# BenChung/SuccessiveConvexification

Measured on AMD Instinct MI355X. Metric: 6-DoF K=50 SCvx iterations/sec (batch), higher is better.
Workload: dtype f64

## Files before the change

successiveconvexification_amd/csrc/scvx_ipm_core.hpp:

```cpp
#pragma once
#include <math.h>
#include <stdint.h>
#include <type_traits>

#if defined(__HIPCC__)
#define SCVX_HD __host__ __device__ __forceinline__
#define SCVX_HD_NI __host__ __device__ __attribute__((noinline))
#else
#define SCVX_HD inline
#define SCVX_HD_NI inline
#endif
#if defined(SCVX_IPM_PROF) && defined(__HIP_DEVICE_COMPILE__)
#define SCVX_TS(v) const unsigned long long v = __builtin_amdgcn_s_memtime()
#define SCVX_TE(v, slot) prof[slot] += (double)(__builtin_amdgcn_s_memtime() - v)
#else
#define SCVX_TS(v)
#define SCVX_TE(v, slot)
#endif
#ifndef SCVX_NODE_QR
#define SCVX_NODE_QR 0
#endif
#ifndef SCVX_STALL_ITERS
#define SCVX_STALL_ITERS 3
#endif
// ... 342 lines not shown
    int status;
    int iters;
    double merit, pobj;
    int warmed;
    int attempts;
};

template <class Ex, class Stor = double, class DStor = Stor, int NU = 3, class FStor = SCVX_FACTOR_T>
struct Solver {
    static_assert(NU == 3 || NU == 5, "control_dim 3 (the reference's live model) or 5 (fin extension)");
    static constexpr int NP = 14 + 2 * NU + 1;
    static constexpr int DSZ = 14 * NP;
    static constexpr int CS = 14 + 2 * NU;
    static constexpr int NXU = 14 + NU;
    static constexpr int HU_SZ = hu_size(NU);
    static constexpr int NODE_SZ = HX_SZ + HU_SZ;
    static constexpr int TW = 14 + 2 * NU;
    static constexpr int TS = NU == 5 ? 26 : 22;
    static constexpr int BPN = 14 * NU;
    static constexpr int NPW = (DSZ + 63) / 64;
    typedef typename gp<Stor>::ptr gptr;
    typedef typename gp<Stor>::cptr cgptr;
    typedef typename gp<DStor>::ptr dptr;
    typedef typename gp<DStor>::cptr dcptr;
    typedef typename gp<double>::cptr cdptr;
    typedef typename gp<FStor>::ptr fptr;
    typedef typename gp<FStor>::cptr cfptr;
    Ex& ex;
    const Consts& C;
    Layout L;
    cdptr xbar, ubar, endpoint;
    dcptr D;
    double rk;
    gptr dk, V, rx, gx, dw, r1, cw, Vbest, tmpv;
    gptr y, ry, dy, r2, cy, tmpy, tmpy2, rp, tq0, tq1;
    gptr S, Z, lam, Wv, Wibz, tmpc, Wirz, sd;
    gptr Wbeta;
    gptr hx, hu;
    fptr Linv, Nf;
    gptr tchain;
    dptr At;
    gptr ys, ytr, ynu;
    gptr ptl, rtr;
    gptr tmpl, tmpl2;
    gptr uhat, lb0;
    gptr wh, Vw, yw, Sw, Zw;
    double h_tr[4], h_nu[4], hrk, hnui;
    double q_tr[2], q_nu[2], q_sg[4], h00s;
    double css, cst, csn, cts, ctt, ctn, cns, cnt_, pny;
    double p_step_frac = SCVX_STEP_FRAC, p_init_shift = SCVX_INIT_SHIFT, p_init_balance = SCVX_INIT_BALANCE;
    bool p_sigma_cube = false;
    double p_mu_floor = 0.25;
    double bigvz[2];
    double bigs[2][6];
    bool bigs_ok;
    double bigvv[2];
    double bigq[2][6];
    double res_nrx2, res_nry2, res_sgy;
    bool tsp;
    double gram[16];
    double gn_pred;
    double bigvx2[2];
#if defined(SCVX_IPM_PROF)
    double prof[32];
#endif
    double cur_gate;

    SCVX_HD Solver(Ex& e, const Consts& c) : ex(e), C(c) {
        L.init(c.K, c.vmax > 0.0, NU);
#if defined(SCVX_IPM_PROF)
        for (int i = 0; i < 32; i++) prof[i] = 0.0;
#endif
    }

    SCVX_HD void carve(gptr w) {
        const int nv = L.nv, ny = L.ny, nc = L.nc, nloc = L.nloc, K = L.K;
        dk = w; w += ny;
        V = w; w += nv; rx = w; w += nv; gx = w; w += nv; dw = w; w += nv; r1 = w; w += nv; cw = w; w += nv;
        Vbest = w; w += nv; tmpv = w; w += nv;
        y = w; w += ny; ry = w; w += ny; dy = w; w += ny; r2 = w; w += ny; cy = w; w += ny; tmpy = w; w += ny; tmpy2 = w; w += ny; rp = w; w += ny; tq0 = w; w += ny; tq1 = w; w += ny;
        S = w; w += nc; Z = w; w += nc; lam = w; w += nc; Wv = w; w += nc;
        Wibz = w; w += nc; tmpc = w; w += nc; Wirz = w; w += nc; sd = w; w += nc;
        Wbeta = w; w += L.ncones;
        hx = w; w += (size_t)(K + 1) * HX_SZ; hu = w; w += (size_t)(K + 1) * HU_SZ;
        Linv = (fptr)w; w += (size_t)K * LINV_SZ; Nf = (fptr)w; w += (size_t)K * 196; At = (dptr)w; w += (size_t)K * 196;
        tchain = w; w += ny;
        ys = w; w += ny; ytr = w; w += ny; ynu = w; w += ny; rtr = w; w += ny; ptl = w; w += nloc;
        tmpl = w; w += nloc; tmpl2 = w; w += nloc;
        uhat = w; w += 3 * (K + 1); lb0 = w; w += (K + 1);
        w += 64;
        wh = w; w += 8; Vw = w; w += nv; yw = w; w += ny; Sw = w; w += nc; Zw = w; w += nc;
    }

    SCVX_HD bool fixed_x(int k, int j) const {
        if (k == 0) return !(j >= 7 && j < 11);
        if (k == L.K) return j != 0;
        return false;
    }
    SCVX_HD bool fixed_u(int k, int c) const { return k == L.K && (c == 1 || c == 2); }

    template <class PH>
    static SCVX_HD double bhu(const double* Dt, int c0, int i, int c, PH h) {
        if (NU == 3 || c < 3) return Dt[14 * c0 + i] * h[c] + Dt[14 * (c0 + 1) + i] * h[3 + c] + Dt[14 * (c0 + 2) + i] * h[6 + c];
        return Dt[14 * (c0 + 3) + i] * h[9 + (c - 3)] + Dt[14 * (c0 + 4) + i] * h[11 + (c - 3)];
    }
    static SCVX_HD double so_elem(const double* T, const double* Bp, int i, int j) {
        double a = -T[TS * i + j];
        SCVX_UNROLL
// ... 294 lines not shown
        each_small<4>(L.o_dp, L.c_dp, L.ndp, f);
        if (with_sg) { each_small<2>(L.o_sg, L.c_sg, 1, f); each_small<1>(L.o_rk, L.c_rk, 1, f); }
    }

    SCVX_HD void identity_scaling() {
        for (int i = ex.lane(); i < L.nc; i += ex.nlanes()) Wv[i] = 0.0;
        ex.sync();
        all_small([&](auto, int off, int c) { Wv[off] = 1.0; Wbeta[c] = 1.0; }, false);
        if (ex.lane() == 0) {
            Wv[L.o_nu] = 1.0; Wv[L.o_tr] = 1.0; Wv[L.o_sg] = 1.0; Wv[L.o_rk] = 1.0;
            Wbeta[L.c_nu] = Wbeta[L.c_tr] = Wbeta[L.c_sg] = Wbeta[L.c_rk] = 1.0;
        }
        bigvv[0] = bigvv[1] = 0.0;
        ex.sync();
    }
    SCVX_HD_NI void W_all(cgptr in, gptr out, bool inverse) {
        SCVX_THIS_LDS();
        SCVX_T0();
        all_small([&](auto Dt_, int off, int c) {
            constexpr int d = decltype(Dt_)::value;
            const double beta = Wbeta[c];
            if (d == 1) out[off] = inverse ? in[off] / beta : in[off] * beta;
            else {
                double xv[d], vv[d], yv[d];
                for (int i = 0; i < d; i++) { xv[i] = in[off + i]; vv[i] = Wv[off + i]; }
                soc_W_small(vv, beta, d, xv, yv, inverse);
                for (int i = 0; i < d; i++) out[off + i] = yv[i];
            }
        }, true);
        big_W(L.o_nu, 14 * L.K + 1, L.c_nu, in, out, inverse);
        big_W(L.o_tr, NXU * (L.K + 1) + 1, L.c_tr, in, out, inverse);
        ex.sync();
        SCVX_T1(8);
    }
    enum { G_GS3 = 0, G_RATE = 1, G_MASS = 2, G_T4 = 3, G_LB = 4, G_SG = 5, G_RK = 6, G_DP = 7, G_FIN = 8 };
    template <int GRP, int D, class F>
    SCVX_HD void each_small_g(int off0, int c0, int n, F&& f) {
        for (int q = ex.lane(); q < n; q += ex.nlanes())
            f(std::integral_constant<int, GRP>(), std::integral_constant<int, D>(), off0 + D * q, c0 + q, q);
    }
    template <class F>
    SCVX_HD void for_small(F&& f) {
        const int K = L.K;
        each_small_g<G_GS3, 3>(L.o_gs, L.c_gs, 2 * K, f);
        each_small_g<G_RATE, 4>(L.o_rate, L.c_rate, K, f);
        each_small_g<G_MASS, 1>(L.o_mass, L.c_mass, K, f);
        each_small_g<G_T4, 4>(L.o_tb, L.c_tb, 2 * (K + 1), f);
        each_small_g<G_LB, 1>(L.o_lb, L.c_lb, K + 1, f);
        if constexpr (NU == 5) each_small_g<G_FIN, 3>(L.o_fin, L.c_fin, L.nfin, f);
        each_small_g<G_DP, 4>(L.o_dp, L.c_dp, L.ndp, f);
        each_small_g<G_SG, 2>(L.o_sg, L.c_sg, 1, f);
        each_small_g<G_RK, 1>(L.o_rk, L.c_rk, 1, f);
    }
    template <int GRP, int D>
    SCVX_HD void small_gather(int q, cgptr v, double af, double (&o)[D]) const {
        const int K = L.K;
        if constexpr (GRP == G_GS3) {
            const bool gs = q < K;
            const int k = gs ? q : q - K;
            cgptr dx = v + 14 * k; cdptr xb = xbar + 14 * k;
            const int i1 = gs ? 2 : 9, i2 = gs ? 3 : 10;
            const double x1 = af * xb[1] + dx[1];
            o[0] = gs ? x1 * C.itan : af * C.sqcm;
            o[1] = af * xb[i1] + dx[i1];
            o[2] = af * xb[i2] + dx[i2];
        } else if constexpr (GRP == G_RATE) {
            cgptr dx = v + 14 * q; cdptr xb = xbar + 14 * q;
            o[0] = af * C.omMax;
            for (int j = 0; j < 3; j++) o[1 + j] = af * xb[11 + j] + dx[11 + j];
        } else if constexpr (GRP == G_MASS) {
            const int k = q + 1;
            o[0] = (af * xbar[14 * k] + v[14 * k]) - af * C.mdry;
        } else if constexpr (GRP == G_T4) {
            const bool tb = q <= K;
            const int k = tb ? q : q - (K + 1);
            cgptr du = v + L.nx + NU * k; cdptr ub = ubar + NU * k;
            double u[3];
            for (int c = 0; c < 3; c++) u[c] = af * ub[c] + du[c];
            o[0] = tb ? af * C.Tmax : u[0] * C.icos;
            o[1] = u[0]; o[2] = u[1]; o[3] = u[2];
        } else if constexpr (GRP == G_LB) {
            cgptr du = v + L.nx + NU * q;
            o[0] = uhat[3 * q] * du[0] + uhat[3 * q + 1] * du[1] + uhat[3 * q + 2] * du[2] - af * lb0[q];
        } else if constexpr (GRP == G_FIN) {
            cgptr du = v + L.nx + NU * q; cdptr ub = ubar + NU * q;
            o[0] = af * C.finmxf;
            o[1] = af * ub[3] + du[3];
            o[2] = af * ub[4] + du[4];
        } else if constexpr (GRP == G_DP) {
            cgptr dx = v + 14 * q; cdptr xb = xbar + 14 * q;
            o[0] = af * C.vmax;
            for (int j = 0; j < 3; j++) o[1 + j] = af * xb[4 + j] + dx[4 + j];
        } else if constexpr (GRP == G_SG) {
            o[0] = v[L.iTS]; o[1] = v[L.iS];
        } else {
            o[0] = af * rk - v[L.iTTR];
        }
    }
    struct BigCone { int off, dim, cidx, head, body; };
    SCVX_HD BigCone big_cone(int q) const {
        return q == 0 ? BigCone{L.o_nu, 14 * L.K + 1, L.c_nu, L.iTNU, L.nx + L.nu_}
                      : BigCone{L.o_tr, NXU * (L.K + 1) + 1, L.c_tr, L.iTTR, 0};
    }
    struct D6 { double a, b, c, d, e, f; };

    SCVX_HD_NI void scale_pass(double& gap_out, double& nrz2_out) {
        SCVX_THIS_LDS();
        SCVX_T0();
        double gap = 0, nrz2 = 0;
        const cgptr S_ = S; const cgptr Z_ = Z; const cgptr V_ = V;
        const gptr Wv_ = Wv; const gptr lam_ = lam; const gptr Wirz_ = Wirz; const gptr tmpc_ = tmpc; const gptr Wbeta_ = Wbeta;
        for_small([&](auto G_, auto Dt_, int off, int c, int q) {
            constexpr int GRP = decltype(G_)::value, D = decltype(Dt_)::value;
            double s[D], z[D], a[D], r[D];
            for (int i = 0; i < D; i++) { s[i] = S_[off + i]; z[i] = Z_[off + i]; }
            small_gather<GRP, D>(q, V_, 1.0, a);
            for (int i = 0; i < D; i++) { r[i] = s[i] - a[i]; gap += s[i] * z[i]; nrz2 += r[i] * r[i]; }
            if constexpr (D == 1) {
                const double beta = sqrt(s[0] / z[0]), l = sqrt(s[0] * z[0]);
                const double wr = r[0] / beta;
                Wbeta_[c] = beta; Wv_[off] = 1.0; lam_[off] = l; Wirz_[off] = wr; tmpc_[off] = (l - wr) / beta;
            } else {
                double beta, v[D], l[D], wr[D], m[D], t[D];
                soc_nt_small(s, z, D, v, beta);
                soc_W_small(v, beta, D, z, l, false);
                soc_W_small(v, beta, D, r, wr, true);
                for (int i = 0; i < D; i++) m[i] = l[i] - wr[i];
                soc_W_small(v, beta, D, m, t, true);
                Wbeta_[c] = beta;
                for (int i = 0; i < D; i++) { Wv_[off + i] = v[i]; lam_[off + i] = l[i]; Wirz_[off + i] = wr[i]; tmpc_[off + i] = t[i]; }
            }
        });
        for (int q = 0; q < 2; q++) {
            const BigCone bc = big_cone(q);
            const cgptr s = S_ + bc.off; const cgptr z = Z_ + bc.off; const cgptr ab = V_ + bc.body - 1;
            double a = 0, b = 0, c = 0;
            const bool carried = SCVX_CARRY_BIGSUMS != 0 && bigs_ok;
            if (carried) { a = bigs[q][0]; b = bigs[q][1]; c = bigs[q][2]; }
            else {
                stream(1, bc.dim, [&](int i) { return D2{s[i], z[i]}; },
                       [&](int, const D2& v) { a += v.a * v.a; b += v.b * v.b; c += v.a * v.b; });
                a = ex.sum(a); b = ex.sum(b); c = ex.sum(c);
            }
            const double s0 = s[0], z0 = z[0], r0 = s0 - V_[bc.head];
            const double sj = sqrt(s0 * s0 - a), zj = sqrt(z0 * z0 - b);
            const double isj = 1.0 / sj, izj = 1.0 / zj;
            const double gam = sqrt(0.5 * (1.0 + (s0 * z0 + c) * isj * izj));
            const double ig = 0.5 / gam;
            const double wb0 = (s0 * isj + z0 * izj) * ig;
            const double den = 1.0 / sqrt(2.0 * (wb0 + 1.0));
            const double v0 = (wb0 + 1.0) * den, beta = sqrt(sj * izj), ibeta = 1.0 / beta;
            const double igd = ig * den;
            double vz = 0, vr = 0, vv = 0, g1 = 0, n1 = 0;
            if (carried) {
                const double sr = bigs[q][3], zr = bigs[q][4];
                vz = (c * isj - b * izj) * igd;
                vr = (sr * isj - zr * izj) * igd;
                vv = ((a * isj) * isj - 2.0 * (c * isj) * izj + (b * izj) * izj) * (igd * igd);
                if (ex.lane() == 0) { gap += c; nrz2 += bigs[q][5]; }
            } else {
            stream(1, bc.dim, [&](int i) { return D3{s[i], z[i], ab[i]}; },
                   [&](int, const D3& w) {
                       const double vi = (w.a * isj - w.b * izj) * igd, ri = w.a - w.c;
                       vz += vi * w.b; vr += vi * ri; vv += vi * vi; g1 += w.a * w.b; n1 += ri * ri;
                   });
            vz = ex.sum(vz); vr = ex.sum(vr); vv = ex.sum(vv);
            }
            bigvv[q] = vv;
            gap += g1; nrz2 += n1;
            if (ex.lane() == 0) { gap += s0 * z0; nrz2 += r0 * r0; }
            const double vxz = v0 * z0 + vz;
            const double l0 = (2.0 * vxz * v0 - z0) * beta;
            const double vxr = v0 * r0 - vr;
            const double wr0 = (2.0 * vxr * v0 - r0) * ibeta;
            const double m0 = l0 - wr0;
            const double vl = beta * (2.0 * vxz * vv + vz);
            const double vw = (-2.0 * vxr * vv + vr) * ibeta;
            const double vxm = v0 * m0 - (vl - vw);
            const double t0 = (2.0 * vxm * v0 - m0) * ibeta;
            const gptr vo = Wv_ + bc.off; const gptr lo = lam_ + bc.off; const gptr wo = Wirz_ + bc.off; const gptr to = tmpc_ + bc.off;
            stream(1, bc.dim, [&](int i) { return D3{s[i], z[i], ab[i]}; },
                   [&](int i, const D3& w) {
                       const double vi = (w.a * isj - w.b * izj) * igd, ri = w.a - w.c;
                       const double li = (2.0 * vxz * vi + w.b) * beta;
                       const double wi = (-2.0 * vxr * vi + ri) * ibeta;
                       vo[i] = vi; lo[i] = li; wo[i] = wi;
                       to[i] = (-2.0 * vxm * vi + (li - wi)) * ibeta;
                   });
            if (ex.lane() == 0) { vo[0] = v0; lo[0] = l0; wo[0] = wr0; to[0] = t0; Wbeta_[bc.cidx] = beta; }
        }
        ex.sync();
        gap_out = ex.sum(gap);
        nrz2_out = ex.sum(nrz2);
        SCVX_T1(11);
    }

    template <bool PRED, bool CHECK = false>
    SCVX_HD_NI double dir_pass() {
        static_assert(!(PRED && CHECK), "the operator-form check belongs to the corrector");
        SCVX_THIS_LDS();
        SCVX_T0();
        double amax = INFINITY;
        const cgptr dw_ = dw; const cgptr Wv_ = Wv; const cgptr lam_ = lam; const cgptr Wirz_ = Wirz; const cgptr Wibz_ = Wibz;
        const cgptr Wbeta_ = Wbeta; const gptr sd_ = sd; const gptr tc_ = tmpc;
        for_small([&](auto G_, auto Dt_, int off, int c, int q) {
            constexpr int GRP = decltype(G_)::value, D = decltype(Dt_)::value;
            double ds[D], l[D], wr[D], a[D], b[D];
            small_gather<GRP, D>(q, dw_, 0.0, ds);
            const double beta = Wbeta_[c];
            for (int i = 0; i < D; i++) { l[i] = lam_[off + i]; wr[i] = Wirz_[off + i]; }
            if constexpr (D == 1) {
                const double wij = ds[0] / beta;
                if (CHECK) tc_[off] = wij / beta;
                a[0] = wij - wr[0];
                b[0] = PRED ? -l[0] - a[0] : -(wij + Wibz_[off]);
                const double sa = a[0] < 0.0 ? -l[0] / a[0] : INFINITY, sb = b[0] < 0.0 ? -l[0] / b[0] : INFINITY;
                if (sa < amax) amax = sa;
                if (sb < amax) amax = sb;
            } else {
                double v[D], wij[D];
                for (int i = 0; i < D; i++) v[i] = Wv_[off + i];
                soc_W_small(v, beta, D, ds, wij, true);
                if (CHECK) {
                    double uu[D];
                    soc_W_small(v, beta, D, wij, uu, true);
                    for (int i = 0; i < D; i++) tc_[off + i] = uu[i];
                }
                for (int i = 0; i < D; i++) { a[i] = wij[i] - wr[i]; b[i] = PRED ? -l[i] - a[i] : -(wij[i] + Wibz_[off + i]); }
                double ll = 0, la = 0, aa = 0, lb = 0, bb = 0;
                for (int i = 1; i < D; i++) { ll += l[i] * l[i]; la += l[i] * a[i]; aa += a[i] * a[i]; lb += l[i] * b[i]; bb += b[i] * b[i]; }
                const double sa = soc_maxstep_parts(l[0], a[0], l[0] * l[0] - ll, l[0] * a[0] - la, a[0] * a[0] - aa);
                const double sb = soc_maxstep_parts(l[0], b[0], l[0] * l[0] - ll, l[0] * b[0] - lb, b[0] * b[0] - bb);
                if (sa < amax) amax = sa;
                if (sb < amax) amax = sb;
            }
            for (int i = 0; i < D; i++) sd_[off + i] = PRED ? a[i] : b[i];
        });
        amax = ex.min(amax);
        for (int q = 0; q < 2; q++) {
            const BigCone bc = big_cone(q);
            const cgptr v = Wv_ + bc.off; const cgptr l = lam_ + bc.off; const cgptr wr = Wirz_ + bc.off; const cgptr wb = Wibz_ + bc.off;
            const cgptr db = dw_ + bc.body - 1;
            const gptr so = sd_ + bc.off;
            double vd = 0;
            stream(1, bc.dim, [&](int i) { return D2{v[i], db[i]}; }, [&](int, const D2& w) { vd += w.a * w.b; });
            vd = ex.sum(vd);
            const double beta = Wbeta_[bc.cidx], ibeta = 1.0 / beta, v0 = v[0], d0 = dw_[bc.head], l0 = l[0];
// ... 51 lines not shown
        const gptr Wibz_ = Wibz; const gptr tmpc_ = tmpc;
        for_small([&](auto, auto Dt_, int off, int c, int) {
            constexpr int D = decltype(Dt_)::value;
            double l[D], a[D], b[D], wr[D];
            for (int i = 0; i < D; i++) { l[i] = lam_[off + i]; a[i] = sd_[off + i]; wr[i] = Wirz_[off + i]; b[i] = -l[i] - a[i]; }
            const double beta = Wbeta_[c];
            if constexpr (D == 1) {
                const double rhs = -l[0] * l[0] + (-a[0] * b[0] + sigmu);
                const double wb = -wr[0] - rhs / l[0];
                Wibz_[off] = wb; tmpc_[off] = wb / beta;
            } else {
                double rhs[D], t[D], wb[D], v[D], o[D];
                double ll = 0, ab = 0;
                for (int i = 0; i < D; i++) { ll += l[i] * l[i]; ab += a[i] * b[i]; }
                for (int i = 1; i < D; i++) rhs[i] = -2.0 * l[0] * l[i] - (a[0] * b[i] + b[0] * a[i]);
                rhs[0] = -ll + (-ab + sigmu);
                double ld = 0, l1 = 0;
                for (int i = 1; i < D; i++) { ld += l[i] * rhs[i]; l1 += l[i] * l[i]; }
                const double x0 = (l[0] * rhs[0] - ld) / (l[0] * l[0] - l1);
                const double il0 = 1.0 / l[0];
                t[0] = x0;
                for (int i = 1; i < D; i++) t[i] = (rhs[i] - x0 * l[i]) * il0;
                for (int i = 0; i < D; i++) { wb[i] = -wr[i] - t[i]; v[i] = Wv_[off + i]; }
                soc_W_small(v, beta, D, wb, o, true);
                for (int i = 0; i < D; i++) { Wibz_[off + i] = wb[i]; tmpc_[off + i] = o[i]; }
            }
        });
        for (int q = 0; q < 2; q++) {
            const BigCone bc = big_cone(q);
            const cgptr v = Wv_ + bc.off; const cgptr l = lam_ + bc.off; const cgptr wr = Wirz_ + bc.off; const cgptr a = sd_ + bc.off;
            const gptr wbo = Wibz_ + bc.off; const gptr to = tmpc_ + bc.off;
            const double l0 = l[0], a0 = a[0], b0 = -l0 - a0, v0 = v[0], wr0 = wr[0];
            const double beta = Wbeta_[bc.cidx], ibeta = 1.0 / beta;
            const double c1 = -2.0 * l0 + a0, c2 = a0 - b0;
            const double ll = bigq[q][0], la = bigq[q][1], aa = bigq[q][2], vl = bigq[q][3], vw = bigq[q][4], va = bigq[q][5];
            const double ab = -la - aa, lr = c1 * ll + c2 * la, vr = c1 * vl + c2 * va;
            const double rhs0 = -(ll + l0 * l0) + (-(ab + a0 * b0) + sigmu);
            const double x0 = (l0 * rhs0 - lr) / (l0 * l0 - ll);
            const double il0 = 1.0 / l0;
            const double wb0 = -wr0 - x0;
            const double vt = (vr - x0 * vl) * il0;
            const double vx = v0 * wb0 - (-vw - vt);
            stream(1, bc.dim, [&](int i) { return D4{l[i], a[i], v[i], wr[i]}; },
                   [&](int i, const D4& w) {
                       const double bi = -w.a - w.b, ri = -2.0 * l0 * w.a - (a0 * bi + b0 * w.b);
                       const double wbi = -w.d - (ri - x0 * w.a) * il0;
                       wbo[i] = wbi;
                       to[i] = (-2.0 * vx * w.c + wbi) * ibeta;
                   });
            if (ex.lane() == 0) { wbo[0] = wb0; to[0] = (2.0 * vx * v0 - wb0) * ibeta; }
        }
        ex.sync();
        SCVX_T1(22);
    }

    SCVX_HD_NI void update_pass(double alpha, gptr Vn) {
        SCVX_THIS_LDS();
        SCVX_T0();
        const gptr S_ = S; const gptr Z_ = Z; const cgptr V_ = V; const cgptr dw_ = dw; const cgptr Wv_ = Wv; const cgptr sd_ = sd;
        const cgptr Wbeta_ = Wbeta;
        for_small([&](auto G_, auto Dt_, int off, int c, int q) {
            constexpr int GRP = decltype(G_)::value, D = decltype(Dt_)::value;
            double s[D], z[D], a[D], jd[D], b[D];
            for (int i = 0; i < D; i++) { s[i] = S_[off + i]; z[i] = Z_[off + i]; b[i] = sd_[off + i]; }
            small_gather<GRP, D>(q, V_, 1.0, a);
            small_gather<GRP, D>(q, dw_, 0.0, jd);
            const double beta = Wbeta_[c];
            if constexpr (D == 1) {
                S_[off] = s[0] + alpha * (jd[0] - (s[0] - a[0]));
                Z_[off] = z[0] + alpha * (b[0] / beta);
            } else {
                double v[D], dz[D];
                for (int i = 0; i < D; i++) v[i] = Wv_[off + i];
                soc_W_small(v, beta, D, b, dz, true);
                for (int i = 0; i < D; i++) { S_[off + i] = s[i] + alpha * (jd[i] - (s[i] - a[i])); Z_[off + i] = z[i] + alpha * dz[i]; }
            }
        });
        for (int q = 0; q < 2; q++) {
            const BigCone bc = big_cone(q);
            const gptr s = S_ + bc.off; const gptr z = Z_ + bc.off; const cgptr v = Wv_ + bc.off; const cgptr b = sd_ + bc.off;
            const cgptr ab = V_ + bc.body - 1; const cgptr db = dw_ + bc.body - 1;
            const double beta = Wbeta_[bc.cidx], ibeta = 1.0 / beta, v0 = v[0], b0 = b[0];
            const double vx = v0 * b0 - bigvz[q];
            const double s0 = s[0], z0 = z[0], a0 = V_[bc.head], d0 = dw_[bc.head];
            ex.sync();
            const gptr vnb = Vn + bc.body - 1;
            double q0 = 0, q1 = 0, q2 = 0, q3 = 0, q4 = 0, q5 = 0;
            stream(1, bc.dim, [&](int i) { return D6{s[i], z[i], v[i], b[i], ab[i], db[i]}; },
                   [&](int i, const D6& w) {
                       const double sn = w.a + alpha * (w.f - (w.a - w.e));
                       const double zn = w.b + alpha * ((-2.0 * vx * w.c + w.d) * ibeta);
                       const double vn = w.e + alpha * w.f;
                       s[i] = sn; z[i] = zn; vnb[i] = vn;
                       const double rn = sn - vn;
                       q0 += sn * sn; q1 += zn * zn; q2 += sn * zn; q3 += sn * rn; q4 += zn * rn; q5 += rn * rn;
                   });
            bigs[q][0] = ex.sum(q0); bigs[q][1] = ex.sum(q1); bigs[q][2] = ex.sum(q2);
            bigs[q][3] = ex.sum(q3); bigs[q][4] = ex.sum(q4); bigs[q][5] = ex.sum(q5);
            if (ex.lane() == 0) {
                s[0] = s0 + alpha * (d0 - (s0 - a0));
                z[0] = z0 + alpha * ((2.0 * vx * v0 - b0) * ibeta);
            }
        }
        ex.sync();
        for (int i = L.nloc + ex.lane(); i < L.nv; i += ex.nlanes()) Vn[i] = V_[i] + alpha * dw_[i];
        bigs_ok = true;
        {
            const gptr y_ = y; const cgptr dy_ = dy;
            stream(0, L.ny, [&](int i) { return D2{y_[i], dy_[i]}; }, [&](int i, const D2& v) { y_[i] = v.a + alpha * v.b; });
        }
        ex.sync();
        SCVX_T1(23);
    }

    SCVX_HD_NI void Hb_inv(cgptr g, gptr out, bool with_nu = true) {
        SCVX_THIS_LDS();
        SCVX_T0();
        const int K = L.K;
        const cgptr hx_ = hx; const cgptr hu_ = hu;
        stream(0, L.nx,
               [&](int t) {
                   const int k = t / 14, j = t - 14 * k;
                   const int hb = j == 0 ? HX_M : j < 4 ? HX_R + 3 * (j - 1) : j < 7 ? HX_V + 3 * (j - 4) : j < 9 ? HX_Q
                                  : j < 11 ? HX_Q34 + 2 * (j - 9) : HX_W + 3 * (j - 11);
                   const int gb = j == 0 ? 0 : j < 4 ? 1 : j < 7 ? 4 : j < 9 ? j : j < 11 ? 9 : 11;
                   const int n = (j == 0 || j == 7 || j == 8) ? 1 : (j == 9 || j == 10) ? 2 : 3;
                   cgptr h = hx_ + (size_t)k * HX_SZ + hb; cgptr x = g + 14 * k + gb;
                   const int i1 = n > 1 ? 1 : 0, i2 = n > 2 ? 2 : 0;
                   return D6{h[0], n > 1 ? h[i1] : 0.0, n > 2 ? h[i2] : 0.0, x[0], x[i1], x[i2]};
               },
               [&](int t, const D6& w) { out[t] = w.a * w.d + w.b * w.e + w.c * w.f; });
        {
            cgptr gu = g + L.nx; gptr ou = out + L.nx;
            stream(0, L.nu_,
                   [&](int t) {
                       const int k = t / NU, c = t - NU * k;
                       if (NU == 3 || c < 3) { cgptr h = hu_ + HU_SZ * k + 3 * c; cgptr x = gu + NU * k; return D6{h[0], h[1], h[2], x[0], x[1], x[2]}; }
                       cgptr h = hu_ + HU_SZ * k + 9 + 2 * (c - 3); cgptr x = gu + NU * k + 3;
                       return D6{h[0], h[1], 0.0, x[0], x[1], 0.0};
                   },
                   [&](int t, const D6& w) { ou[t] = w.a * w.d + w.b * w.e + w.c * w.f; });
        }
        if (with_nu) {
            cgptr gn = g + L.nx + L.nu_; gptr on = out + L.nx + L.nu_;
            const double hn = hnui;
            stream<8>(0, 14 * K, [&](int i) { return gn[i]; }, [&](int i, double v) { on[i] = hn * v; });
        }
        ex.sync();
        SCVX_T1(3);
    }

    SCVX_HD bool twisted() const { return Ex::kTwisted && L.K >= 8; }
    template <int N>
    SCVX_HD void chains_fwd(const cgptr (&tz)[N], const gptr (&x)[N]) {
        const int K = L.K;
        const cfptr Nf = this->Nf;
        if constexpr (Ex::kTwisted) {
            if (twisted()) {
                const int m = K / 2;
                ex.template chain_range_n<N>(0, K, tz, Nf, x, false, 0, m, true);
                ex.template chain_range_n<N>(2, K, tz, Nf, x, true, K - 1, K - 1 - m, true);
                ex.sync();
                for (int e = ex.lane(); e < 14 * N; e += ex.nlanes()) {
                    const int q = e / 14, i = e - 14 * q;
                    cfptr Na = Nf + (size_t)m * 196 + i;
// ... 1967 lines not shown
            cdptr u = ubar + NU * k;
            const double un = sqrt(u[0] * u[0] + u[1] * u[1] + u[2] * u[2]);
            for (int c = 0; c < 3; c++) uhat[3 * k + c] = u[c] / un;
            lb0[k] = C.Tmin - un;
        }
        ex.sync();
        Result res;
        int iters_all = 0, first_warmed = 0;
        const gptr V_first = V, Vbest_first = Vbest;
        for (int attempt = 0;; attempt++) {
            V = V_first; Vbest = Vbest_first;
            const double r_step[8] = {SCVX_STEP_FRAC,   0.9,  0.95, SCVX_STEP_FRAC, 0.8, 0.9, 0.85, 0.7};
            const double r_shift[8] = {SCVX_INIT_SHIFT, SCVX_INIT_SHIFT, SCVX_INIT_SHIFT, 1.0, SCVX_INIT_SHIFT, 5.0, 2.0, 0.5};
            const double r_bal[8] = {SCVX_INIT_BALANCE, SCVX_INIT_BALANCE, SCVX_INIT_BALANCE, 0.5, SCVX_INIT_BALANCE, SCVX_INIT_BALANCE, 0.5, 2.0};
            const double r_floor[8] = {0.25, 0.25, 0.25, 0.25, 0.5, 0.25, 0.25, 0.5};
            const int a = attempt < 8 ? attempt : 7;
            p_step_frac = r_step[a]; p_init_shift = r_shift[a]; p_init_balance = r_bal[a]; p_mu_floor = r_floor[a];
            p_sigma_cube = a == 2 || a == 6;
            res = attempt_solve(ic, warm && attempt == 0);
            iters_all += res.iters;
            if (attempt == 0) first_warmed = res.warmed;
            if (!(res.status >= 1 && res.status <= 3) || attempt >= C.retries) { res.attempts = attempt + 1; break; }
            SCVX_DBG("attempt %d ended with status %d at merit %.3e: next rule\n", attempt, res.status, res.merit);
        }
        res.iters = iters_all; res.warmed = first_warmed;
        SCVX_TE(tTot_, 15);
        return res;
    }

    SCVX_HD_NI Result attempt_solve(cdptr ic, bool warm) {
        SCVX_THIS_LDS();
        const int K = L.K;
        zero(V, L.nv); zero(y, L.ny);
        if (ex.lane() == 0) {
            V[0] = C.mwet - xbar[0];
            for (int i = 0; i < 3; i++) { V[1 + i] = ic[i] - xbar[1 + i]; V[4 + i] = ic[3 + i] - xbar[4 + i]; V[11 + i] = C.wBi[i] - xbar[11 + i]; }
            cdptr xK = xbar + 14 * K;
            gptr vK = V + 14 * K;
            for (int i = 0; i < 3; i++) { vK[1 + i] = C.rIf[i] - xK[1 + i]; vK[4 + i] = C.vIf[i] - xK[4 + i]; vK[11 + i] = C.wBf[i] - xK[11 + i]; }
            for (int i = 0; i < 4; i++) vK[7 + i] = C.qBIf[i] - xK[7 + i];
            V[L.nx + NU * K + 1] = 0.0 - ubar[NU * K + 1];
            V[L.nx + NU * K + 2] = 0.0 - ubar[NU * K + 2];
        }
        ex.sync();
        Result res; res.status = 1; res.iters = 0; res.merit = INFINITY; res.pobj = 0; res.warmed = 0; res.attempts = 1;
        {
            const double r1 = ic[0], r2 = ic[1], r3 = ic[2];
            bool bad = sqrt(r2 * r2 + r3 * r3) > r1 * C.itan * (1.0 + 1e-12) + 1e-14;
            bad = bad || sqrt(C.wBi[0] * C.wBi[0] + C.wBi[1] * C.wBi[1] + C.wBi[2] * C.wBi[2]) > C.omMax * (1.0 + 1e-12);
            if (C.vmax > 0.0) bad = bad || sqrt(ic[3] * ic[3] + ic[4] * ic[4] + ic[5] * ic[5]) > C.vmax * (1.0 + 1e-12);
            if (bad) { res.status = 5; return res; }
        }
        cur_gate = INFINITY;
        bigs_ok = false;
        const bool warmed = warm && wh[0] == 1.0 && Vw[L.iTTR] < SCVX_WARM_RADIUS * rk;
        const bool blend = warm && wh[0] == 1.0 && !warmed;
        res.warmed = warmed ? 1 : 0;
        if (warmed) {
            copy(V, Vw, L.nv); copy(y, yw, L.ny); copy(S, Sw, L.nc); copy(Z, Zw, L.nc);
            if (ex.lane() == 0) {
                const double srk = rk - V[L.iTTR], flo = 1e-3 * rk;
                S[L.o_rk] = srk > flo ? srk : flo;
            }
            ex.sync();
        } else {
        ex.sync();
        if (ex.lane() == 0) wh[0] = 0.0;
        identity_scaling();
        if (!build_kkt()) { res.status = 2; return res; }
        cone_map(V, S, true);
        cone_map_t(S, gx);
        for (int i = ex.lane(); i < L.nv; i += ex.nlanes()) gx[i] = -gx[i];
        ex.sync();
        mask_fixed(gx);
        E_apply(V, ry, true);
        for (int i = ex.lane(); i < L.ny; i += ex.nlanes()) r2[i] = -(ry[i] + dk[i]);
        ex.sync();
        kkt_solve(gx, r2, dw, dy);
        for (int i = ex.lane(); i < L.nv; i += ex.nlanes()) V[i] += dw[i];
        ex.sync();
        cone_map(V, S, true);
        zero(gx, L.nv);
        if (ex.lane() == 0) { gx[14 * K] = 1.0; gx[L.iTNU] = -C.wNu; gx[L.iTTR] = -0.5; gx[L.iTS] = -1.0; }
        ex.sync();
        mask_fixed(gx);
        zero(r2, L.ny);
        kkt_solve(gx, r2, dw, y);
        cone_map(dw, Z, false);
        for (int i = ex.lane(); i < L.nc; i += ex.nlanes()) Z[i] = -Z[i];
        ex.sync();
        SCVX_DBG("init: |V|^2 %.12e s %.6e tnu %.6e ttr %.6e ts %.6e |y|^2 %.6e |S|^2 %.12e |Z|^2 %.6e\n", dot(V, V, L.nv), V[L.iS], V[L.iTNU], V[L.iTTR], V[L.iTS], dot(y, y, L.ny), dot(S, S, L.nc), dot(Z, Z, L.nc));
        shift_into_cone(S);
        shift_into_cone(Z);
        if (p_init_balance > 0.0) {
            const double sz = dot(S, Z, L.nc);
            double es = 0, ez = 0;
            all_small([&](auto, int off, int) { es += S[off]; ez += Z[off]; }, true);
            if (ex.lane() == 0) { es += S[L.o_nu] + S[L.o_tr]; ez += Z[L.o_nu] + Z[L.o_tr]; }
            es = ex.sum(es); ez = ex.sum(ez);
            const double dsh = p_init_balance * sz / ez, dzh = p_init_balance * sz / es;
            ex.sync();
            all_small([&](auto, int off, int) { S[off] += dsh; Z[off] += dzh; }, true);
            if (ex.lane() == 0) { S[L.o_nu] += dsh; S[L.o_tr] += dsh; Z[L.o_nu] += dzh; Z[L.o_tr] += dzh; }
            ex.sync();
        }
        SCVX_DBG("shifted: |S|^2 %.12e |Z|^2 %.12e\n", dot(S, S, L.nc), dot(Z, Z, L.nc));
        if (blend && SCVX_BLEND_WARM > 0.0) {
            const double lm = SCVX_BLEND_WARM, th = SCVX_BLEND_RADIUS * rk / Vw[L.iTTR];
            cone_map(V, tmpc, true);
            for (int i = ex.lane(); i < L.nc; i += ex.nlanes()) tmpc[i] = S[i] - tmpc[i];
            ex.sync();
            for (int i = ex.lane(); i < L.nv; i += ex.nlanes()) {
                bool fx = false;
                if (i < 14) fx = fixed_x(0, i); else if (i >= 14 * K && i < L.nx) fx = fixed_x(K, i - 14 * K);
                else if (i == L.nx + NU * K + 1 || i == L.nx + NU * K + 2) fx = true;
                if (!fx) V[i] = lm * th * Vw[i] + (1.0 - lm) * V[i];
            }
            for (int i = ex.lane(); i < L.ny; i += ex.nlanes()) y[i] = lm * yw[i] + (1.0 - lm) * y[i];
            ex.sync();
            cone_map(V, S, true);
            for (int i = ex.lane(); i < L.nc; i += ex.nlanes()) { S[i] += (1.0 - lm) * tmpc[i]; Z[i] = lm * Zw[i] + (1.0 - lm) * Z[i]; }
            ex.sync();
        }
        }

        double best_merit = INFINITY; int best_it = 0;
        bool best_in_V = false;
        bool kept = false;
        const int degree = L.ncones;
        bool res_carried = false;
        double nrx_c = 0.0, nry_c = 0.0;
        for (int it = 1; it <= C.max_iter; it++) {
            res.iters = it;
            double gap, nrz2;
            scale_pass(gap, nrz2);
            SCVX_TS(tR_);
            const bool fused = SCVX_FUSED_RES != 0 && Ex::kFusedResidual && !(warmed && it == 1);
            double nrx, nry;
            bool kkt_ok = true;
            auto eval_residuals = [&]() {
                cone_map_t(Z, rx);
                double nrx2 = 0.0;
                const double sgy = Et_apply(y, rx, rx, 2, 0.0, 0.0, nullptr, &nrx2);
                const double g0 = -rx[L.iS] + sgy, g1 = C.wNu - rx[L.iTNU], g2 = 0.5 - rx[L.iTTR], g3 = 1.0 - rx[L.iTS];
                ex.sync();
                if (ex.lane() == 0) { rx[L.iS] = g0; rx[L.iTNU] = g1; rx[L.iTTR] = g2; rx[L.iTS] = g3; }
                ex.sync();
                const double nry2 = E_apply(V, ry, true, dk, 1.0);
                nrx = sqrt(nrx2 + (g0 * g0 + g1 * g1 + g2 * g2 + g3 * g3)); nry = sqrt(nry2);
            };
            if (!fused) {
                if (res_carried) { nrx = nrx_c; nry = nry_c; }
                else eval_residuals();
            } else {
                cone_map_t(Z, rx, nullptr, false, true);
                if (ex.lane() == 0) {
                    rx[14 * K] += -1.0;
                    rx[L.iTNU] = C.wNu + rx[L.iTNU];
                    rx[L.iTTR] = 0.5 + rx[L.iTTR];
                    rx[L.iTS] = 1.0 + rx[L.iTS];
                }
                ex.sync();
                cone_map_t(tmpc, gx, rx);
                kkt_ok = build_kkt(true, true);
                if (ex.lane() == 0) { rx[L.iS] += res_sgy; gx[L.iS] -= res_sgy; }
                ex.sync();
                const double g0 = rx[L.iS], g1 = rx[L.iTNU], g2 = rx[L.iTTR], g3 = rx[L.iTS];
                nrx = sqrt(res_nrx2 + (g0 * g0 + g1 * g1 + g2 * g2 + g3 * g3)); nry = sqrt(res_nry2);
            }
            const double pobj = -V[14 * K] + C.wNu * V[L.iTNU] + 0.5 * V[L.iTTR] + V[L.iTS];
            const double nrz = sqrt(nrz2);
            const double relgap = gap / (fabs(pobj) > 1.0 ? fabs(pobj) : 1.0);
            double pres = nry > nrz ? nry : nrz;
            double dres = nrx / (C.wNu > 1.0 ? C.wNu : 1.0);
            double merit = pres > dres ? pres : dres;
            if (relgap > merit) merit = relgap;
            if (res_carried && !(merit >= SCVX_RESID_FRESH_FROM)) {
                eval_residuals();
                res_carried = false;
                pres = nry > nrz ? nry : nrz;
                dres = nrx / (C.wNu > 1.0 ? C.wNu : 1.0);
                merit = pres > dres ? pres : dres;
                if (relgap > merit) merit = relgap;
            }
            SCVX_TE(tR_, 9);
            SCVX_DBG("%3d pobj %+.8e gap %.2e pres %.2e (ry %.2e rz %.2e) dres %.2e\n", it, pobj, gap, pres, nry, nrz, dres);
            if (!(merit == merit) || !(gap == gap)) { res.status = 3; break; }
            cur_gate = pres > relgap ? pres : relgap;
            if (merit < best_merit) {
                best_merit = merit; best_it = it; res.pobj = pobj;
                best_in_V = true;
                ex.sync();
            }
            if (!kept && merit < SCVX_WARM_SAVE * C.tol) {
                copy(Vw, V, L.nv); copy(yw, y, L.ny); copy(Sw, S, L.nc); copy(Zw, Z, L.nc);
                if (ex.lane() == 0) wh[0] = 1.0;
                ex.sync();
                kept = true;
            }
            if (pres < C.tol && dres < C.tol && relgap < C.tol) { res.status = 0; break; }
            auto stop_status = [&](int why) { return best_merit < C.tol ? 0 : (best_merit < C.accept ? 4 : why); };
            if (best_merit < C.accept && merit > SCVX_BLOWUP_STOP * best_merit) { res.status = stop_status(2); break; }
            if (it - best_it >= SCVX_STALL_ITERS && best_merit < 1e-5) { res.status = stop_status(2); break; }
            if (it == C.max_iter) { res.status = stop_status(1); break; }
            if (!fused) {
                cone_map_t(tmpc, gx, rx, false, false, true);
                kkt_ok = build_kkt(true);
            }
            if (!kkt_ok) { SCVX_DBG("    factorisation failed\n"); res.status = stop_status(2); break; }
            const double mu = gap / degree;
            { SCVX_TS(tN_); newton_solve(true); SCVX_TE(tN_, 10); }
            double alpha = dir_pass<true>();
            if (alpha > 1.0) alpha = 1.0;
            const double om = 1.0 - alpha;
            const double sig = p_sigma_cube ? om * om * om : (om * om) * (om * om);
            SCVX_DBG("    aff alpha %.6e |dw|^2 %.6e ds %.6e dtnu %.6e dttr %.6e\n", alpha, dot(dw, dw, L.nv), dw[L.iS], dw[L.iTNU], dw[L.iTTR]);
            double smu = sig * mu;
#ifndef SCVX_MU_FLOOR
#define SCVX_MU_FLOOR 0.25
#endif
            {
                const double apo = fabs(pobj) > 1.0 ? fabs(pobj) : 1.0;
                const double mu_floor = p_mu_floor * C.tol * apo / degree;
                if (smu < mu_floor) smu = mu_floor < mu ? mu_floor : mu;
#if defined(SCVX_HOLD_MU)
                if (relgap < C.tol && pres < C.tol) smu = mu;
#endif
            }
            corr_rhs_pass(smu);
#if SCVX_REFINE_FUSED
            { SCVX_TS(tN_); alpha = p_step_frac * newton_corr(); SCVX_TE(tN_, 10); }
#else
            { SCVX_TS(tN_); newton_solve(false); SCVX_TE(tN_, 10); }
            alpha = p_step_frac * dir_pass<false>();
#endif
            if (alpha > 1.0) alpha = 1.0;
            SCVX_DBG("    cmb alpha %.6e |dw|^2 %.6e\n", alpha, dot(dw, dw, L.nv));
            if (!(alpha == alpha)) { res.status = stop_status(3); break; }
            if (alpha < 1e-9) { res.status = stop_status(2); break; }
            {
                const gptr Vn = best_in_V ? Vbest : V;
                update_pass(alpha, Vn);
                if (best_in_V) { Vbest = V; V = Vn; best_in_V = false; }
            }
            res_carried = false;
            if (SCVX_RESID_UPDATE != 0 && !fused && merit >= SCVX_RESID_FRESH_FROM && (it & 7) != 0) {
                const double om = 1.0 - alpha;
                {
                    gptr rx_ = rx; gptr ry_ = ry;
                    stream(0, L.nv, [&](int i) { return rx_[i]; }, [&](int i, double v) { rx_[i] = om * v; });
                    stream(0, L.ny, [&](int i) { return ry_[i]; }, [&](int i, double v) { ry_[i] = om * v; });
                }
                ex.sync();
                nrx_c = om * nrx; nry_c = om * nry;
                res_carried = true;
            }
        }
        res.merit = best_merit;
        if (best_it > 0 && !best_in_V) V = Vbest;
        return res;
    }
};

}
}
```

Before: 148,800.

## Fuse iterate update with next-iteration NT scaling and residual rescale

Merges the update pass with the following iteration's scaling pass into one sweep. The updated S/Z/V values are consumed directly to recompute the Nesterov-Todd scalings, lambda and related quantities, which removes a separate kernel pass, its syncs and a reload of S/Z. The carried residual scaling (rx, ry times 1-alpha) is folded into the same streams instead of running as extra passes. This adds code complexity and templated branching, and small cones gather V+alpha*dw inline rather than reading it back from memory.

```diff
diff --git a/successiveconvexification_amd/csrc/scvx_ipm_core.hpp b/successiveconvexification_amd/csrc/scvx_ipm_core.hpp
--- a/successiveconvexification_amd/csrc/scvx_ipm_core.hpp
+++ b/successiveconvexification_amd/csrc/scvx_ipm_core.hpp
@@ -418,8 +418,6 @@
     bool p_sigma_cube = false;
     double p_mu_floor = 0.25;
     double bigvz[2];
-    double bigs[2][6];
-    bool bigs_ok;
     double bigvv[2];
     double bigq[2][6];
     double res_nrx2, res_nry2, res_sgy;
@@ -820,50 +818,54 @@
         each_small_g<G_SG, 2>(L.o_sg, L.c_sg, 1, f);
         each_small_g<G_RK, 1>(L.o_rk, L.c_rk, 1, f);
     }
-    template <int GRP, int D>
-    SCVX_HD void small_gather(int q, cgptr v, double af, double (&o)[D]) const {
+    template <int GRP, int D, class A>
+    SCVX_HD void small_gather_at(int q, A&& at, double af, double (&o)[D]) const {
         const int K = L.K;
         if constexpr (GRP == G_GS3) {
             const bool gs = q < K;
             const int k = gs ? q : q - K;
-            cgptr dx = v + 14 * k; cdptr xb = xbar + 14 * k;
+            const int dx = 14 * k; cdptr xb = xbar + 14 * k;
             const int i1 = gs ? 2 : 9, i2 = gs ? 3 : 10;
-            const double x1 = af * xb[1] + dx[1];
+            const double x1 = af * xb[1] + at(dx + 1);
             o[0] = gs ? x1 * C.itan : af * C.sqcm;
-            o[1] = af * xb[i1] + dx[i1];
-            o[2] = af * xb[i2] + dx[i2];
+            o[1] = af * xb[i1] + at(dx + i1);
+            o[2] = af * xb[i2] + at(dx + i2);
         } else if constexpr (GRP == G_RATE) {
-            cgptr dx = v + 14 * q; cdptr xb = xbar + 14 * q;
+            const int dx = 14 * q; cdptr xb = xbar + 14 * q;
             o[0] = af * C.omMax;
-            for (int j = 0; j < 3; j++) o[1 + j] = af * xb[11 + j] + dx[11 + j];
+            for (int j = 0; j < 3; j++) o[1 + j] = af * xb[11 + j] + at(dx + 11 + j);
         } else if constexpr (GRP == G_MASS) {
             const int k = q + 1;
-            o[0] = (af * xbar[14 * k] + v[14 * k]) - af * C.mdry;
+            o[0] = (af * xbar[14 * k] + at(14 * k)) - af * C.mdry;
         } else if constexpr (GRP == G_T4) {
             const bool tb = q <= K;
             const int k = tb ? q : q - (K + 1);
-            cgptr du = v + L.nx + NU * k; cdptr ub = ubar + NU * k;
+            const int du = L.nx + NU * k; cdptr ub = ubar + NU * k;
             double u[3];
-            for (int c = 0; c < 3; c++) u[c] = af * ub[c] + du[c];
+            for (int c = 0; c < 3; c++) u[c] = af * ub[c] + at(du + c);
             o[0] = tb ? af * C.Tmax : u[0] * C.icos;
             o[1] = u[0]; o[2] = u[1]; o[3] = u[2];
         } else if constexpr (GRP == G_LB) {
-            cgptr du = v + L.nx + NU * q;
-            o[0] = uhat[3 * q] * du[0] + uhat[3 * q + 1] * du[1] + uhat[3 * q + 2] * du[2] - af * lb0[q];
+            const int du = L.nx + NU * q;
+            o[0] = uhat[3 * q] * at(du) + uhat[3 * q + 1] * at(du + 1) + uhat[3 * q + 2] * at(du + 2) - af * lb0[q];
         } else if constexpr (GRP == G_FIN) {
-            cgptr du = v + L.nx + NU * q; cdptr ub = ubar + NU * q;
+            const int du = L.nx + NU * q; cdptr ub = ubar + NU * q;
             o[0] = af * C.finmxf;
-            o[1] = af * ub[3] + du[3];
-            o[2] = af * ub[4] + du[4];
+            o[1] = af * ub[3] + at(du + 3);
+            o[2] = af * ub[4] + at(du + 4);
         } else if constexpr (GRP == G_DP) {
-            cgptr dx = v + 14 * q; cdptr xb = xbar + 14 * q;
+            const int dx = 14 * q; cdptr xb = xbar + 14 * q;
             o[0] = af * C.vmax;
-            for (int j = 0; j < 3; j++) o[1 + j] = af * xb[4 + j] + dx[4 + j];
+            for (int j = 0; j < 3; j++) o[1 + j] = af * xb[4 + j] + at(dx + 4 + j);
         } else if constexpr (GRP == G_SG) {
-            o[0] = v[L.iTS]; o[1] = v[L.iS];
+            o[0] = at(L.iTS); o[1] = at(L.iS);
         } else {
-            o[0] = af * rk - v[L.iTTR];
-        }
+            o[0] = af * rk - at(L.iTTR);
+        }
+    }
+    template <int GRP, int D>
+    SCVX_HD void small_gather(int q, cgptr v, double af, double (&o)[D]) const {
+        small_gather_at<GRP, D>(q, [&](int i) { return v[i]; }, af, o);
     }
     struct BigCone { int off, dim, cidx, head, body; };
     SCVX_HD BigCone big_cone(int q) const {
@@ -872,17 +874,42 @@
     }
     struct D6 { double a, b, c, d, e, f; };
 
-    SCVX_HD_NI void scale_pass(double& gap_out, double& nrz2_out) {
+    template <bool UPD>
+    SCVX_HD_NI void iterate_sweep(double alpha, gptr Vn, double om_res, double& gap_out, double& nrz2_out) {
+        constexpr bool SUMS6 = SCVX_CARRY_BIGSUMS != 0;
         SCVX_THIS_LDS();
         SCVX_T0();
         double gap = 0, nrz2 = 0;
-        const cgptr S_ = S; const cgptr Z_ = Z; const cgptr V_ = V;
+        const gptr S_ = S; const gptr Z_ = Z; const cgptr V_ = V; const cgptr dw_ = dw; const cgptr sd_ = sd;
         const gptr Wv_ = Wv; const gptr lam_ = lam; const gptr Wirz_ = Wirz; const gptr tmpc_ = tmpc; const gptr Wbeta_ = Wbeta;
+        const gptr rx_ = rx;
+        const bool sres = UPD && om_res >= 0.0;
+        const auto vnew = [&](int i) { return V_[i] + alpha * dw_[i]; };
         for_small([&](auto G_, auto Dt_, int off, int c, int q) {
             constexpr int GRP = decltype(G_)::value, D = decltype(Dt_)::value;
-            double s[D], z[D], a[D], r[D];
-            for (int i = 0; i < D; i++) { s[i] = S_[off + i]; z[i] = Z_[off + i]; }
-            small_gather<GRP, D>(q, V_, 1.0, a);
+            double s[D], z[D], a[D];
+            if constexpr (UPD) {
+                double so[D], zo[D], ao[D], jd[D], b[D];
+                for (int i = 0; i < D; i++) { so[i] = S_[off + i]; zo[i] = Z_[off + i]; b[i] = sd_[off + i]; }
+                small_gather<GRP, D>(q, V_, 1.0, ao);
+                small_gather<GRP, D>(q, dw_, 0.0, jd);
+                const double beta = Wbeta_[c];
+                if constexpr (D == 1) {
+                    s[0] = so[0] + alpha * (jd[0] - (so[0] - ao[0]));
+                    z[0] = zo[0] + alpha * (b[0] / beta);
+                } else {
+                    double v[D], dz[D];
+                    for (int i = 0; i < D; i++) v[i] = Wv_[off + i];
+                    soc_W_small(v, beta, D, b, dz, true);
+                    for (int i = 0; i < D; i++) { s[i] = so[i] + alpha * (jd[i] - (so[i] - ao[i])); z[i] = zo[i] + alpha * dz[i]; }
+                }
+                small_gather_at<GRP, D>(q, vnew, 1.0, a);
+                for (int i = 0; i < D; i++) { S_[off + i] = s[i]; Z_[off + i] = z[i]; }
+            } else {
+                for (int i = 0; i < D; i++) { s[i] = S_[off + i]; z[i] = Z_[off + i]; }
+                small_gather<GRP, D>(q, V_, 1.0, a);
+            }
+            double r[D];
             for (int i = 0; i < D; i++) { r[i] = s[i] - a[i]; gap += s[i] * z[i]; nrz2 += r[i] * r[i]; }
             if constexpr (D == 1) {
                 const double beta = sqrt(s[0] / z[0]), l = sqrt(s[0] * z[0]);
@@ -901,16 +928,43 @@
         });
         for (int q = 0; q < 2; q++) {
             const BigCone bc = big_cone(q);
-            const cgptr s = S_ + bc.off; const cgptr z = Z_ + bc.off; const cgptr ab = V_ + bc.body - 1;
-            double a = 0, b = 0, c = 0;
-            const bool carried = SCVX_CARRY_BIGSUMS != 0 && bigs_ok;
-            if (carried) { a = bigs[q][0]; b = bigs[q][1]; c = bigs[q][2]; }
-            else {
+            const gptr s = S_ + bc.off; const gptr z = Z_ + bc.off;
+            const cgptr ab = (UPD ? (cgptr)Vn : V_) + bc.body - 1;
+            double a = 0, b = 0, c = 0, sr = 0, zr = 0, rr = 0;
+            double s0, z0, r0;
+            bool carried;
+            if constexpr (UPD) {
+                const cgptr v = Wv_ + bc.off; const cgptr bd = sd_ + bc.off;
+                const cgptr abo = V_ + bc.body - 1; const cgptr db = dw_ + bc.body - 1;
+                const double beta = Wbeta_[bc.cidx], ibeta = 1.0 / beta, v0 = v[0], b0 = bd[0];
+                const double vx = v0 * b0 - bigvz[q];
+                const double so0 = s[0], zo0 = z[0], a0 = V_[bc.head], d0 = dw_[bc.head];
+                ex.sync();
+                const gptr vnb = Vn + bc.body - 1;
+                double q0 = 0, q1 = 0, q2 = 0, q3 = 0, q4 = 0, q5 = 0;
+                stream(1, bc.dim, [&](int i) { return D6{s[i], z[i], v[i], bd[i], abo[i], db[i]}; },
+                       [&](int i, const D6& w) {
+                           const double sn = w.a + alpha * (w.f - (w.a - w.e));
+                           const double zn = w.b + alpha * ((-2.0 * vx * w.c + w.d) * ibeta);
+                           const double vn = w.e + alpha * w.f;
+                           s[i] = sn; z[i] = zn; vnb[i] = vn;
+                           q0 += sn * sn; q1 += zn * zn; q2 += sn * zn;
+                           if constexpr (SUMS6) { const double rn = sn - vn; q3 += sn * rn; q4 += zn * rn; q5 += rn * rn; }
+                       });
+                s0 = so0 + alpha * (d0 - (so0 - a0));
+                z0 = zo0 + alpha * ((2.0 * vx * v0 - b0) * ibeta);
+                r0 = s0 - (a0 + alpha * d0);
+                if (ex.lane() == 0) { s[0] = s0; z[0] = z0; }
+                a = ex.sum(q0); b = ex.sum(q1); c = ex.sum(q2);
+                if constexpr (SUMS6) { sr = ex.sum(q3); zr = ex.sum(q4); rr = ex.sum(q5); }
+                carried = SUMS6;
+            } else {
+                carried = false;
                 stream(1, bc.dim, [&](int i) { return D2{s[i], z[i]}; },
                        [&](int, const D2& v) { a += v.a * v.a; b += v.b * v.b; c += v.a * v.b; });
                 a = ex.sum(a); b = ex.sum(b); c = ex.sum(c);
-            }
-            const double s0 = s[0], z0 = z[0], r0 = s0 - V_[bc.head];
+                s0 = s[0]; z0 = z[0]; r0 = s0 - V_[bc.head];
+            }
             const double sj = sqrt(s0 * s0 - a), zj = sqrt(z0 * z0 - b);
             const double isj = 1.0 / sj, izj = 1.0 / zj;
             const double gam = sqrt(0.5 * (1.0 + (s0 * z0 + c) * isj * izj));
@@ -921,18 +975,17 @@
             const double igd = ig * den;
             double vz = 0, vr = 0, vv = 0, g1 = 0, n1 = 0;
             if (carried) {
-                const double sr = bigs[q][3], zr = bigs[q][4];
                 vz = (c * isj - b * izj) * igd;
                 vr = (sr * isj - zr * izj) * igd;
                 vv = ((a * isj) * isj - 2.0 * (c * isj) * izj + (b * izj) * izj) * (igd * igd);
-                if (ex.lane() == 0) { gap += c; nrz2 += bigs[q][5]; }
+                if (ex.lane() == 0) { gap += c; nrz2 += rr; }
             } else {
-            stream(1, bc.dim, [&](int i) { return D3{s[i], z[i], ab[i]}; },
-                   [&](int, const D3& w) {
-                       const double vi = (w.a * isj - w.b * izj) * igd, ri = w.a - w.c;
-                       vz += vi * w.b; vr += vi * ri; vv += vi * vi; g1 += w.a * w.b; n1 += ri * ri;
-                   });
-            vz = ex.sum(vz); vr = ex.sum(vr); vv = ex.sum(vv);
+                stream(1, bc.dim, [&](int i) { return D3{s[i], z[i], ab[i]}; },
+                       [&](int, const D3& w) {
+                           const double vi = (w.a * isj - w.b * izj) * igd, ri = w.a - w.c;
+                           vz += vi * w.b; vr += vi * ri; vv += vi * vi; g1 += w.a * w.b; n1 += ri * ri;
+                       });
+                vz = ex.sum(vz); vr = ex.sum(vr); vv = ex.sum(vv);
             }
             bigvv[q] = vv;
             gap += g1; nrz2 += n1;
@@ -947,20 +1000,35 @@
             const double vxm = v0 * m0 - (vl - vw);
             const double t0 = (2.0 * vxm * v0 - m0) * ibeta;
             const gptr vo = Wv_ + bc.off; const gptr lo = lam_ + bc.off; const gptr wo = Wirz_ + bc.off; const gptr to = tmpc_ + bc.off;
-            stream(1, bc.dim, [&](int i) { return D3{s[i], z[i], ab[i]}; },
-                   [&](int i, const D3& w) {
+            const gptr rb = rx_ + bc.body - 1;
+            stream(1, bc.dim, [&](int i) { return D4{s[i], z[i], ab[i], sres ? rb[i] : 0.0}; },
+                   [&](int i, const D4& w) {
                        const double vi = (w.a * isj - w.b * izj) * igd, ri = w.a - w.c;
                        const double li = (2.0 * vxz * vi + w.b) * beta;
                        const double wi = (-2.0 * vxr * vi + ri) * ibeta;
                        vo[i] = vi; lo[i] = li; wo[i] = wi;
                        to[i] = (-2.0 * vxm * vi + (li - wi)) * ibeta;
+                       if (sres) rb[i] = om_res * w.d;
                    });
             if (ex.lane() == 0) { vo[0] = v0; lo[0] = l0; wo[0] = wr0; to[0] = t0; Wbeta_[bc.cidx] = beta; }
         }
         ex.sync();
+        if constexpr (UPD) {
+            for (int i = L.nloc + ex.lane(); i < L.nv; i += ex.nlanes()) {
+                Vn[i] = V_[i] + alpha * dw_[i];
+                if (sres) rx_[i] = om_res * rx_[i];
+            }
+            {
+                const gptr y_ = y; const cgptr dy_ = dy; const gptr ry_ = ry;
+                if (sres) stream(0, L.ny, [&](int i) { return D3{y_[i], dy_[i], ry_[i]}; },
+                                 [&](int i, const D3& v) { y_[i] = v.a + alpha * v.b; ry_[i] = om_res * v.c; });
+                else stream(0, L.ny, [&](int i) { return D2{y_[i], dy_[i]}; }, [&](int i, const D2& v) { y_[i] = v.a + alpha * v.b; });
+            }
+            ex.sync();
+        }
         gap_out = ex.sum(gap);
         nrz2_out = ex.sum(nrz2);
-        SCVX_T1(11);
+        SCVX_T1(UPD ? 19 : 11);
     }
 
     template <bool PRED, bool CHECK = false>
@@ -1118,65 +1186,6 @@
         }
         ex.sync();
         SCVX_T1(22);
-    }
-
-    SCVX_HD_NI void update_pass(double alpha, gptr Vn) {
-        SCVX_THIS_LDS();
-        SCVX_T0();
-        const gptr S_ = S; const gptr Z_ = Z; const cgptr V_ = V; const cgptr dw_ = dw; const cgptr Wv_ = Wv; const cgptr sd_ = sd;
-        const cgptr Wbeta_ = Wbeta;
-        for_small([&](auto G_, auto Dt_, int off, int c, int q) {
-            constexpr int GRP = decltype(G_)::value, D = decltype(Dt_)::value;
-            double s[D], z[D], a[D], jd[D], b[D];
-            for (int i = 0; i < D; i++) { s[i] = S_[off + i]; z[i] = Z_[off + i]; b[i] = sd_[off + i]; }
-            small_gather<GRP, D>(q, V_, 1.0, a);
-            small_gather<GRP, D>(q, dw_, 0.0, jd);
-            const double beta = Wbeta_[c];
-            if constexpr (D == 1) {
-                S_[off] = s[0] + alpha * (jd[0] - (s[0] - a[0]));
-                Z_[off] = z[0] + alpha * (b[0] / beta);
-            } else {
-                double v[D], dz[D];
-                for (int i = 0; i < D; i++) v[i] = Wv_[off + i];
-                soc_W_small(v, beta, D, b, dz, true);
-                for (int i = 0; i < D; i++) { S_[off + i] = s[i] + alpha * (jd[i] - (s[i] - a[i])); Z_[off + i] = z[i] + alpha * dz[i]; }
-            }
-        });
-        for (int q = 0; q < 2; q++) {
-            const BigCone bc = big_cone(q);
-            const gptr s = S_ + bc.off; const gptr z = Z_ + bc.off; const cgptr v = Wv_ + bc.off; const cgptr b = sd_ + bc.off;
-            const cgptr ab = V_ + bc.body - 1; const cgptr db = dw_ + bc.body - 1;
-            const double beta = Wbeta_[bc.cidx], ibeta = 1.0 / beta, v0 = v[0], b0 = b[0];
-            const double vx = v0 * b0 - bigvz[q];
-            const double s0 = s[0], z0 = z[0], a0 = V_[bc.head], d0 = dw_[bc.head];
-            ex.sync();
-            const gptr vnb = Vn + bc.body - 1;
-            double q0 = 0, q1 = 0, q2 = 0, q3 = 0, q4 = 0, q5 = 0;
-            stream(1, bc.dim, [&](int i) { return D6{s[i], z[i], v[i], b[i], ab[i], db[i]}; },
-                   [&](int i, const D6& w) {
-                       const double sn = w.a + alpha * (w.f - (w.a - w.e));
-                       const double zn = w.b + alpha * ((-2.0 * vx * w.c + w.d) * ibeta);
-                       const double vn = w.e + alpha * w.f;
-                       s[i] = sn; z[i] = zn; vnb[i] = vn;
-                       const double rn = sn - vn;
-                       q0 += sn * sn; q1 += zn * zn; q2 += sn * zn; q3 += sn * rn; q4 += zn * rn; q5 += rn * rn;
-                   });
-            bigs[q][0] = ex.sum(q0); bigs[q][1] = ex.sum(q1); bigs[q][2] = ex.sum(q2);
-            bigs[q][3] = ex.sum(q3); bigs[q][4] = ex.sum(q4); bigs[q][5] = ex.sum(q5);
-            if (ex.lane() == 0) {
-                s[0] = s0 + alpha * (d0 - (s0 - a0));
-                z[0] = z0 + alpha * ((2.0 * vx * v0 - b0) * ibeta);
-            }
-        }
-        ex.sync();
-        for (int i = L.nloc + ex.lane(); i < L.nv; i += ex.nlanes()) Vn[i] = V_[i] + alpha * dw_[i];
-        bigs_ok = true;
-        {
-            const gptr y_ = y; const cgptr dy_ = dy;
-            stream(0, L.ny, [&](int i) { return D2{y_[i], dy_[i]}; }, [&](int i, const D2& v) { y_[i] = v.a + alpha * v.b; });
-        }
-        ex.sync();
-        SCVX_T1(23);
     }
 
     SCVX_HD_NI void Hb_inv(cgptr g, gptr out, bool with_nu = true) {
@@ -3250,7 +3259,6 @@
             if (bad) { res.status = 5; return res; }
         }
         cur_gate = INFINITY;
-        bigs_ok = false;
         const bool warmed = warm && wh[0] == 1.0 && Vw[L.iTTR] < SCVX_WARM_RADIUS * rk;
         const bool blend = warm && wh[0] == 1.0 && !warmed;
         res.warmed = warmed ? 1 : 0;
@@ -3328,10 +3336,10 @@
         const int degree = L.ncones;
         bool res_carried = false;
         double nrx_c = 0.0, nry_c = 0.0;
+        double gap = 0.0, nrz2 = 0.0;
         for (int it = 1; it <= C.max_iter; it++) {
             res.iters = it;
-            double gap, nrz2;
-            scale_pass(gap, nrz2);
+            if (it == 1) iterate_sweep<false>(0.0, V, -1.0, gap, nrz2);
             SCVX_TS(tR_);
             const bool fused = SCVX_FUSED_RES != 0 && Ex::kFusedResidual && !(warmed && it == 1);
             double nrx, nry;
@@ -3436,23 +3444,14 @@
             SCVX_DBG("    cmb alpha %.6e |dw|^2 %.6e\n", alpha, dot(dw, dw, L.nv));
             if (!(alpha == alpha)) { res.status = stop_status(3); break; }
             if (alpha < 1e-9) { res.status = stop_status(2); break; }
+            res_carried = SCVX_RESID_UPDATE != 0 && !fused && merit >= SCVX_RESID_FRESH_FROM && (it & 7) != 0;
+            const double om_res = 1.0 - alpha;
             {
                 const gptr Vn = best_in_V ? Vbest : V;
-                update_pass(alpha, Vn);
+                iterate_sweep<true>(alpha, Vn, res_carried ? om_res : -1.0, gap, nrz2);
                 if (best_in_V) { Vbest = V; V = Vn; best_in_V = false; }
             }
-            res_carried = false;
-            if (SCVX_RESID_UPDATE != 0 && !fused && merit >= SCVX_RESID_FRESH_FROM && (it & 7) != 0) {
-                const double om = 1.0 - alpha;
-                {
-                    gptr rx_ = rx; gptr ry_ = ry;
-                    stream(0, L.nv, [&](int i) { return rx_[i]; }, [&](int i, double v) { rx_[i] = om * v; });
-                    stream(0, L.ny, [&](int i) { return ry_[i]; }, [&](int i, double v) { ry_[i] = om * v; });
-                }
-                ex.sync();
-                nrx_c = om * nrx; nry_c = om * nry;
-                res_carried = true;
-            }
+            if (res_carried) { nrx_c = om_res * nrx; nry_c = om_res * nry; }
         }
         res.merit = best_merit;
         if (best_it > 0 && !best_in_V) V = Vbest;
```

Result: no change. 151,300, median of 6 (+1.7%).
